# arkworks-rs/groth16

Hardware: AMD Instinct MI355X
Metric: R1CS constraints/sec (create_proof, BLS12-381) (higher is better)
Workload: dtype u32-limb Montgomery integers (Fr 255-bit, Fq 381-bit); 1 GPU; SYN(k=22) synthetic R1CS, 4194302 constraints, FFT domain 2^22, bls12_381, full create_proof (7 NTTs + 4 G1 MSMs + 1 G2 MSM), valid proving key generated on the GPU from seeded toxic waste; curve=bls12_381, log2_domain=22, constraints=4194302, key=valid, witness=resident in HBM at entry (--full: value_incl_h2d holds the PCIe-inclusive rates), parallelism=single-gpu

## Files before the change

groth16_amd/csrc/fp30.hpp:

```cpp
#pragma once
#include "field.hpp"
#include "fips_asm_gen.hpp"

#if defined(__HIP_DEVICE_COMPILE__) && !defined(G16_NO_FIPS_ASM)
#define G16_ASM_PRODUCTS 1
#endif

namespace g16 {

template <class P>
struct Fp30 {
    typedef P Params_t;
    static constexpr int NL = P::NL30;
    static constexpr int NW = P::N;
    static constexpr uint32_t MASK = (1u << 30) - 1u;
    uint32_t l[NL];

    G16_HD static Fp30 zero() {
        Fp30 r;
        G16_UNROLL for (int i = 0; i < NL; ++i) r.l[i] = 0;
        return r;
    }
    G16_HD static Fp30 one() {
        Fp30 r;
// ... 351 lines not shown
        }
        Fp30 r;
        const bool lt = br < 0;
        G16_UNROLL for (int i = 0; i < NL; ++i) r.l[i] = lt ? l[i] : d.l[i];
        return r;
    }
    G16_HD Fp30 weak_reduce32() const { return cond_sub<16>().template cond_sub<8>().template cond_sub<4>().template cond_sub<2>(); }
    G16_HD bool raw_zero() const {
        uint32_t a = 0;
        G16_UNROLL for (int i = 0; i < NL; ++i) a |= l[i];
        return a == 0;
    }
    typedef Fp30 Raw;
    static constexpr int KM = 2, K2M = 4, KX = 8, KY = 4;
#ifndef G16_ACC_MIN_WAVES
#define G16_ACC_MIN_WAVES 2
#endif
    static constexpr int ACC_MIN_WAVES = G16_ACC_MIN_WAVES;
    static constexpr bool ACC_PREFETCH = true;
    static constexpr int LANES_PER_TASK = 1;
    template <class A>
    G16_HD static bool load_point(const A* bases, int64_t idx, Fp30& px, Fp30& py) {
        const A p = bases[idx];
        if (p.is_identity()) return false;
        px = from_packed(p.x);
        py = from_packed(p.y);
        return true;
    }
    template <class A>
    G16_HD static bool load_point_py(const A* bases, int64_t idx, Fp30& px, PackedC& yw) {
        const A p = bases[idx];
        if (p.is_identity()) return false;
        px = from_packed(p.x);
        yw = p.y;
        return true;
    }


    G16_HD Fp30 canonical_lt2p() const {
        Fp30 d;
        int32_t br = 0;
        G16_UNROLL for (int i = 0; i < NL; ++i) {
            const int32_t v = (int32_t)l[i] - (int32_t)P::p30(i) + br;
            if (i == NL - 1) { d.l[i] = (uint32_t)v; br = v >> 31; }
            else { d.l[i] = (uint32_t)v & MASK; br = v >> 30; }
        }
        Fp30 r;
        const bool lt = br < 0;
        G16_UNROLL for (int i = 0; i < NL; ++i) r.l[i] = lt ? l[i] : d.l[i];
        return r;
    }

    G16_HD Fp30 canonical_lt8p() const { return cond_sub<4>().template cond_sub<2>().canonical_lt2p(); }
    G16_HD Fp30 canonical_quick() const {
        constexpr uint32_t D = P::p30(NL - 1) + 1u;
        static_assert(D > (1u << 13), "the top limb of p carries at least 14 bits for every supported field");
        constexpr uint64_t MAGIC = ((uint64_t)1 << 40) / D;
        const uint32_t q = (uint32_t)(((uint64_t)l[NL - 1] * MAGIC) >> 40);
        Fp30 r;
        int64_t carry = 0;
        G16_UNROLL for (int i = 0; i < NL; ++i) {
            const int64_t t = (int64_t)l[i] - (int64_t)((uint64_t)q * P::p30(i)) + carry;
            r.l[i] = (i == NL - 1) ? (uint32_t)t : ((uint32_t)t & MASK);
            carry = t >> 30;
        }
        return r.canonical_lt8p();
    }
    G16_HD Fp30 neg_canonical() const {
        Fp30 d;
        int32_t br = 0;
        G16_UNROLL for (int i = 0; i < NL; ++i) {
            const int32_t v = (int32_t)P::p30(i) - (int32_t)l[i] + br;
            if (i == NL - 1) d.l[i] = (uint32_t)v;
            else { d.l[i] = (uint32_t)v & MASK; br = v >> 30; }
        }
        return d;
    }
    G16_HD bool same_limbs(const Fp30& o) const {
        uint32_t a = 0;
        G16_UNROLL for (int i = 0; i < NL; ++i) a |= l[i] ^ o.l[i];
        return a == 0;
    }
    static constexpr int PREFIX_LIMBS = NL;
    G16_HD void get_limbs(uint32_t* w) const { G16_UNROLL for (int i = 0; i < NL; ++i) w[i] = l[i]; }
    G16_HD static Fp30 from_limbs(const uint32_t* w) { Fp30 r; G16_UNROLL for (int i = 0; i < NL; ++i) r.l[i] = w[i]; return r; }
    G16_HD bool equals_canonical(const Fp30& o) const { return same_limbs(o); }
    template <class A>
    G16_HD static void store_point(A* dst, int64_t idx, const Fp30& x, const Fp30& y, bool identity) {
        A p;
        if (identity) { p = A::identity(); }
        else { x.pack(p.x.v); y.pack(p.y.v); }
        dst[idx] = p;
    }

    G16_HD Std to_packed() const {
        Std r;
        mul_impl(one()).canonical_lt2p().pack(r.v);
        return r;
    }
    G16_HD static Fp<P> std_to_r30(const Fp<P>& x) {
        Fp<P> c;
        G16_UNROLL for (int i = 0; i < P::N; ++i) c.v[i] = P::r30_plain(i);
        return x * c;
    }
    G16_HD Fp<P> to_std() const {
        Fp30 c;
// ... 548 lines not shown
```

groth16_amd/csrc/hosttest.hip:

```cpp
#include "internal.hpp"
#include "fp30.hpp"
#include "batch_affine.hpp"
#include "window_tables.hpp"
#include "fixed_base.hpp"
#include <cstdlib>
#include <vector>

using namespace g16;

namespace g16 {
template <class P>
struct Fp2e30 {
    typedef Fp30<P> B;
    typedef Fp2p30<P> PP;
    B c0, c1;
    static Fp2e30 one() { return {B::one(), B::zero()}; }
    Fp2e30 add(const Fp2e30& o) const { return {c0.add(o.c0), c1.add(o.c1)}; }
    Fp2e30 dbl() const { return {c0.dbl(), c1.dbl()}; }
    template <int K> Fp2e30 sub(const Fp2e30& o) const { return {c0.template sub<K>(o.c0), c1.template sub<K>(o.c1)}; }
    Fp2e30 mul(const Fp2e30& o) const { return {PP::pair_mul(false, c0, c1, o.c0, o.c1), PP::pair_mul(true, c1, c0, o.c1, o.c0)}; }
    Fp2e30 sqr() const { return {PP::pair_sqr(false, c0, c1), PP::pair_sqr(true, c1, c0)}; }
};
template <class P>
Fp2e30<P> batch_inverse(const Fp2e30<P>& a) { return {pair_inverse<P>(false, a.c0, a.c1), pair_inverse<P>(true, a.c1, a.c0)}; }
// ... 87 lines not shown
    }
    static Fq rand_fq(uint64_t& st) {
        Fq acc = Fq::zero();
        const Fq two64 = Fq::from_u64(1ULL << 32).sqr();
        for (int k = 0; k < 8; ++k) acc = acc * two64 + Fq::from_u64(sm_next(st));
        return acc;
    }
    typedef Fp30<typename Fq::Params> F30;
    static F30 to30(const Fq& x) { const Fq t = F30::std_to_r30(x); return F30::unpack(t.v); }
    static Fr rand_fr(uint64_t& st) {
        Fr acc = Fr::zero();
        const Fr two64 = Fr::from_u64(1ULL << 32).sqr();
        for (int k = 0; k < 8; ++k) acc = acc * two64 + Fr::from_u64(sm_next(st));
        return acc;
    }
    static int selftest_fr30(uint64_t seed, int iters) {
        typedef Fp30<typename Fr::Params> R30;
        uint64_t st = seed ^ 0xF7;
        {
            R30 pl, kp = R30::zero();
            for (int i = 0; i < R30::NL; ++i) pl.l[i] = Fr::Params::p30(i);
            R30 pm1 = pl;
            pm1.l[0] -= 1;
            R30 one_raw = R30::zero();
            one_raw.l[0] = 1;
            for (int k = 0; k <= 5000; ++k) {
                if (k % 7 == 0 || k < 40 || (k & (k - 1)) == 0 || ((k + 1) & k) == 0) {
                    if (!kp.canonical_quick().same_limbs(R30::zero())) return 520;
                    if (!kp.add(pm1).canonical_quick().same_limbs(pm1)) return 521;
                    if (!kp.add(one_raw).canonical_quick().same_limbs(one_raw)) return 522;
                }
                kp = kp.add(pl);
            }
        }
        for (int it = 0; it < iters; ++it) {
            Fr x = rand_fr(st), y = rand_fr(st), w = rand_fr(st);
            if (it == 0) { x = Fr::zero(); }
            if (it == 1) { x = Fr::zero() - Fr::one(); y = x; w = x; }
            const R30 a = R30::unpack(x.v), b = R30::unpack(y.v);
            const Fr wt = R30::std_to_r30(w);
            const R30 w30 = R30::unpack(wt.v);
            auto canon = [](const R30& v) { Fr o; v.mul_impl(R30::one()).canonical_lt2p().pack(o.v); return o; };
            auto quick = [](const R30& v) { Fr o; v.canonical_quick().pack(o.v); return o; };
            if (!(canon(a.mul_impl(w30)) == x * w)) return 501;
            if (!(quick(a.mul_impl(w30)) == x * w) || !(quick(a) == x) || !(quick(R30::zero()) == Fr::zero())) return 505;
            {
                R30 m = R30::unpack((Fr::zero() - Fr::one()).v);
                Fr want = Fr::zero() - Fr::one();
                for (int k = 0; k < 12; ++k) {
                    if (!(quick(m) == want) || !(quick(m.add(R30::unpack(Fr::one().v))) == want + Fr::one())) return 506;
                    m = m.dbl(); want = want + want;
                }
            }
            R30 u = a, v = b;
            Fr ru = x, rv = y;
            for (int k = 0; k < 11; ++k) {
                const R30 t = v.mul_impl(w30);
                const R30 nu = u.add(t), nv = u.template sub<2>(t);
                const Fr rt = rv * w;
                const Fr rnu = ru + rt, rnv = ru - rt;
                u = nu; v = nv; ru = rnu; rv = rnv;
            }
            if (!(canon(u) == ru) || !(canon(v) == rv)) return 502;
            if (!(quick(u) == ru) || !(quick(v) == rv)) return 507;
            u = a; v = b; ru = x; rv = y;
            R30 s2 = a, d2 = b;
            for (int k = 0; k < 11; ++k) {
                const R30 nu = u.add(v);
                const R30 nv = u.sub_pow2(v, k).mul_impl(w30);
                const Fr rnu = ru + rv, rnv = (ru - rv) * w;
                s2 = nu; d2 = nv;
                u = nu; v = nu.add(nv).sub_pow2(nv, k + 1 < 12 ? k + 1 : 11);
                ru = rnu; rv = rnu;
                if (!(canon(d2) == rnv)) return 503;
                if (!(quick(d2) == rnv) || !(quick(nu) == rnu) || !(quick(v) == rnu)) return 508;
            }
            if (!(canon(s2) == ru)) return 504;
        }
        return 0;
    }

    template <class X, class A>
    static int selftest_fixed_base(const A& gen, uint64_t seed, int first_code) {
        uint64_t st = seed ^ 0xFB;
        uint32_t k0[8];
        for (int i = 0; i < 8; ++i) k0[i] = (uint32_t)sm_next(st);
        k0[7] &= 0x0fffffffu;
        const X p = X::from_affine(gen).mul_bits(k0, 256);
        FixedBaseTable<X> tab;
        tab.build(p);
        for (int it = 0; it < 6; ++it) {
            uint32_t k[8];
            for (int i = 0; i < 8; ++i) k[i] = it == 0 ? 0u : it == 1 ? (i == 0 ? 1u : 0u) : it == 2 ? 0xffffffffu : (uint32_t)sm_next(st);
            if (it == 3) for (int i = 0; i < Fr::N; ++i) k[i] = Fr::Params::mod(i) - (i == 0 ? 1u : 0u);
            const auto want = p.mul_bits(k, 256).to_affine();
            if (!(tab.mul(k).to_affine() == want)) return first_code;
            if (!(mul_window4(p, k).to_affine() == want)) return first_code + 1;
        }
        return 0;
    }

    template <class R30>
    static int selftest_columns(uint64_t seed, int iters) {
        typedef unsigned __int128 U128;
        uint64_t st = seed ^ 0xC0;
        for (int it = 0; it < iters + 4; ++it) {
// ... 495 lines not shown
```

groth16_amd/csrc/internal.hpp:

```cpp
#pragma once
#include <hip/hip_runtime.h>
#include <atomic>
#include <cstdint>
#include <cstdio>
#include <cstring>
#include <string>
#include <vector>
#include "../../include/g16_mi355x.h"
#include "curve.hpp"

namespace g16 {

void set_last_error(const char* what, hipError_t e, const char* file, int line);

#define G16_HIP_TRY(expr)                                                     \
    do {                                                                      \
        hipError_t e__ = (expr);                                              \
        if (e__ != hipSuccess) {                                              \
            ::g16::set_last_error(#expr, e__, __FILE__, __LINE__);            \
            return e__ == hipErrorOutOfMemory ? G16_ERR_OOM : G16_ERR_HIP;    \
        }                                                                     \
    } while (0)

#define G16_TRY(expr)                  \
// ... 4 lines not shown

#define G16_LAUNCH_CHECK() G16_HIP_TRY(hipGetLastError())

struct PerDeviceOnce {
    std::atomic<bool> done[64] = {};
    std::atomic<bool>& flag() {
        int dev = 0;
        (void)hipGetDevice(&dev);
        return done[dev & 63];
    }
};

struct Arena {
    struct Chunk { char* p; size_t cap; size_t used; };
    std::vector<Chunk> chunks;
    size_t min_chunk = (size_t)256 << 20;
    void reset() { for (auto& c : chunks) c.used = 0; }
    int alloc(size_t bytes, void** out);
    template <class T> int alloc_n(size_t n, T** out) { return alloc(n * sizeof(T), (void**)out); }
    void release();
    size_t total() const { size_t t = 0; for (auto& c : chunks) t += c.cap; return t; }
};

struct EventTimer {
    hipEvent_t a = nullptr, b = nullptr;
    bool used = false;
    int start(hipStream_t s) {
        if (!a) { G16_HIP_TRY(hipEventCreate(&a)); G16_HIP_TRY(hipEventCreate(&b)); }
        used = true;
        G16_HIP_TRY(hipEventRecord(a, s));
        return G16_OK;
    }
    int stop(hipStream_t s) { G16_HIP_TRY(hipEventRecord(b, s)); return G16_OK; }
    double ms() {
        if (!used) return 0.0;
        float t = 0.f;
        if (hipEventElapsedTime(&t, a, b) != hipSuccess) return 0.0;
        return (double)t;
    }
    void destroy() { if (a) { (void)hipEventDestroy(a); (void)hipEventDestroy(b); a = b = nullptr; } }
};

template <class C>
struct Domain {
    typedef typename C::Fr Fr;
    int log_n = 0;
    size_t n = 0;
    Fr* tw_fwd = nullptr;
    Fr* tw_inv = nullptr;
    Fr* s1_br = nullptr;
    Fr* s2 = nullptr;
    Fr* g_pow = nullptr;
    Fr n_inv, zinv;
};
template <class C> int domain_create(int log_n, hipStream_t st, Domain<C>** out);
template <class C> void domain_destroy(Domain<C>* d);
template <class C> int domain_ensure_gpow(Domain<C>* d, hipStream_t st);

template <class C> int ntt_dif(const Domain<C>* d, typename C::Fr* data, bool inverse, hipStream_t st);
template <class C> int ntt_dif_quotient(const Domain<C>* d, typename C::Fr* a, const typename C::Fr* b, const typename C::Fr* c,
                                        const typename C::Fr& zinv, bool inverse, hipStream_t st);
template <class C> int ntt_dit(const Domain<C>* d, typename C::Fr* data, bool inverse, const typename C::Fr* prescale, hipStream_t st);
template <class C> int ntt_dif_dit(const Domain<C>* d, typename C::Fr* data, bool dif_inverse, const typename C::Fr* prescale, hipStream_t st);
template <class C> int ntt_dif_batch(const Domain<C>* d, typename C::Fr* const* data, int nbatch, bool inverse, hipStream_t st);
template <class C> int ntt_dit_batch(const Domain<C>* d, typename C::Fr* const* data, int nbatch, bool inverse, const typename C::Fr* prescale,
                                     hipStream_t st);
template <class C> int ntt_dif_dit_batch(const Domain<C>* d, typename C::Fr* const* data, int nbatch, bool dif_inverse,
                                         const typename C::Fr* prescale, hipStream_t st);
template <class C> int bitrev_scale(const Domain<C>* d, typename C::Fr* out, const typename C::Fr* in, const typename C::Fr* table,
                                    const typename C::Fr* cst, hipStream_t st);
template <class C> int scale_by_table(typename C::Fr* data, const typename C::Fr* table, size_t n, hipStream_t st);
template <class C> int gen_power_table(typename C::Fr* out, size_t n, const typename C::Fr& base, const typename C::Fr& scale, bool r30_form,
                                       hipStream_t st);

template <class C>
struct DeviceCircuit {
    typedef typename C::Fr Fr;
    uint64_t num_inputs = 0, num_constraints = 0, num_variables = 0;
    uint64_t* row_ptr[3] = {nullptr, nullptr, nullptr};
    uint32_t* col[3] = {nullptr, nullptr, nullptr};
    Fr* val[3] = {nullptr, nullptr, nullptr};
    uint64_t nnz[3] = {0, 0, 0};
    Domain<C>* dom = nullptr;
    static constexpr int Z_CHUNKS = 8;
    uint64_t need_col[Z_CHUNKS] = {};
};
struct ZUpload {
    const void* host = nullptr;
    hipStream_t copy_stream = nullptr;
    hipEvent_t landed[8] = {};
    int pieces = 0;
};
template <class C> int mark_unit_coefficients(DeviceCircuit<C>* ck, hipStream_t st);
template <class C> int witness_map_device(const DeviceCircuit<C>* ck, const typename C::Fr* d_z, typename C::Fr* d_h, Arena& arena,
                                          hipStream_t st, EventTimer* ntt_timers = nullptr, ZUpload* up = nullptr);

template <class C>
struct DistWm {
    typedef typename C::Fr Fr;
    int rank = 0, world = 1, log_world = 0;
    size_t M = 0, blk = 0;
    Domain<C>* dom_m = nullptr;
    Fr* tw1 = nullptr;
    Fr* sc_mid = nullptr;
    Fr* tw2 = nullptr;
    Fr* sc_out = nullptr;
    Fr wn_fwd[8], wn_inv[8];
    Fr zinv;
};
template <class C> int dwm_create(const DeviceCircuit<C>* ck, int rank, int world, hipStream_t st, DistWm<C>** out);
template <class C> void dwm_destroy(DistWm<C>* d);
template <class C> int dwm_stage(const DeviceCircuit<C>* ck, const DistWm<C>* dw, int stage, const typename C::Fr* d_z,
                                 typename C::Fr* const work[3], typename C::Fr* const recv[3], typename C::Fr* h_local, hipStream_t st);

struct MsmPlan {
    int c = 0;
    int W = 0;
    int groups = 0;
    bool merged = false;
    uint32_t B = 0;
    uint32_t Lmax = 0;
    int affine_levels = 0;
    uint32_t chunk = 0;
// ... 75 lines not shown
```

groth16_amd/csrc/ntt.hip:

```cpp
#include "internal.hpp"
#include "fp30.hpp"

namespace g16 {

#ifndef G16_NTT_TILE_LOG
#define G16_NTT_TILE_LOG 10
#endif
static constexpr int NTT_TILE_LOG = G16_NTT_TILE_LOG;
static constexpr int NTT_TILE = 1 << NTT_TILE_LOG;
#ifdef G16_NTT_THREADS
static constexpr int NTT_THREADS = G16_NTT_THREADS;
#else
static constexpr int NTT_THREADS = NTT_TILE_LOG >= 12 ? 512 : 256;
#endif
#ifndef G16_NTT_MAX_R
#define G16_NTT_MAX_R 2
#endif
static constexpr int NTT_MAX_R = G16_NTT_MAX_R;
#ifndef G16_NTT_MIN_WAVES
#define G16_NTT_MIN_WAVES 4
#endif
static constexpr int NTT_MAX_STRIDED = NTT_TILE_LOG >= 12 ? 10 : 8;
static constexpr int NTT_ROW = NTT_TILE + NTT_TILE / 32;

// ... 85 lines not shown
        G16_UNROLL for (int j = 0; j < NE; ++j) {
            const uint32_t c = lds_col(ebase | ((uint32_t)j << p0));
            G16_UNROLL for (int l = 0; l < NL; ++l) lds[l * NTT_ROW + c] = x[j].l[l];
        }
    }
}

template <class P>
struct NttBatch { Fp<P>* p[3]; };
template <class P>
struct NttQuot { const Fp<P>* b; const Fp<P>* c; Fp<P> zinv; };

template <class P, bool DIT>
__global__ __launch_bounds__(NTT_THREADS, G16_NTT_MIN_WAVES) void ntt30_pass_kernel(NttBatch<P> batch, const Tw<P>* __restrict__ tw,
                                                                 const Fp<P>* __restrict__ prescale, int log_n, int s_lo, int s_hi,
                                                                 int T, NttQuot<P> quot) {
    typedef Fp30<P> F;
    constexpr int NL = F::NL;
    extern __shared__ __attribute__((aligned(16))) unsigned char smem[];
    uint32_t* lds = reinterpret_cast<uint32_t*>(smem);
    Fp<P>* __restrict__ data = batch.p[blockIdx.y];
    const int K = s_hi - s_lo;
    const int TT = (s_lo == 0) ? 0 : T;
    const uint32_t E = 1u << (K + TT);
    const uint64_t blk = blockIdx.x;
    uint64_t base;
    if (s_lo == 0) {
        base = blk << K;
    } else {
        const int mid_bits = s_lo - T;
        const uint64_t lowpart = blk & ((1ull << mid_bits) - 1);
        const uint64_t hipart = blk >> mid_bits;
        base = (lowpart << T) | (hipart << s_hi);
    }
    auto gidx = [&](uint32_t e) -> uint64_t {
        if (s_lo == 0) return base + e;
        const uint32_t low = e & ((1u << T) - 1), mid = e >> T;
        return base + low + ((uint64_t)mid << s_lo);
    };
    auto lds_load = [&](uint32_t e) -> F {
        F x;
        const uint32_t c = lds_col(e);
        G16_UNROLL for (int l = 0; l < NL; ++l) x.l[l] = lds[l * NTT_ROW + c];
        return x;
    };
    auto lds_store = [&](uint32_t e, const F& x) {
        const uint32_t c = lds_col(e);
        G16_UNROLL for (int l = 0; l < NL; ++l) lds[l * NTT_ROW + c] = x.l[l];
    };
    for (uint32_t e = threadIdx.x; e < E; e += NTT_THREADS) {
        const uint64_t g = gidx(e);
        F x;
        if (quot.b) {
            const Fp<P> t = (data[g] * quot.b[g] - quot.c[g]) * quot.zinv;
            x = F::unpack(t.v);
        } else {
            x = F::unpack(data[g].v);
        }
        if (prescale) x = x.mul_impl(F::unpack(prescale[g].v));
        lds_store(e, x);
    }
    __syncthreads();
    int done = 0;
    while (done < K) {
        const int R = (K - done) >= NTT_MAX_R ? NTT_MAX_R : (K - done);
        const int q0 = DIT ? done : (K - done - R);
        if (R == 3) ntt30_round<P, DIT, 3>(lds, tw, log_n, s_lo, q0, TT, E, done, gidx, true);
        else if (R == 2) ntt30_round<P, DIT, 2>(lds, tw, log_n, s_lo, q0, TT, E, done, gidx, true);
        else ntt30_round<P, DIT, 1>(lds, tw, log_n, s_lo, q0, TT, E, done, gidx, true);
        __syncthreads();
        done += R;
    }
    for (uint32_t e = threadIdx.x; e < E; e += NTT_THREADS) {
        const F x = lds_load(e).canonical_quick();
        Fp<P> o;
        x.pack(o.v);
        data[gidx(e)] = o;
    }
}

template <class P>
__global__ __launch_bounds__(NTT_THREADS, G16_NTT_MIN_WAVES) void ntt30_dif_dit_kernel(NttBatch<P> batch, const Tw<P>* __restrict__ tw_dif,
                                                                    const Tw<P>* __restrict__ tw_dit, const Fp<P>* __restrict__ prescale,
                                                                    int log_n, int K) {
    typedef Fp30<P> F;
    constexpr int NL = F::NL;
    extern __shared__ __attribute__((aligned(16))) unsigned char smem[];
    uint32_t* lds = reinterpret_cast<uint32_t*>(smem);
    Fp<P>* __restrict__ data = batch.p[blockIdx.y];
    const uint32_t E = 1u << K;
    const uint64_t base = (uint64_t)blockIdx.x << K;
    auto gidx = [&](uint32_t e) -> uint64_t { return base + e; };
    for (uint32_t e = threadIdx.x; e < E; e += NTT_THREADS) {
        const F x = F::unpack(data[base + e].v);
        const uint32_t c = lds_col(e);
        G16_UNROLL for (int l = 0; l < NL; ++l) lds[l * NTT_ROW + c] = x.l[l];
    }
    __syncthreads();
    for (int done = 0; done < K;) {
        const int R = (K - done) >= NTT_MAX_R ? NTT_MAX_R : (K - done);
        const int q0 = K - done - R;
        if (R == 3) ntt30_round<P, false, 3>(lds, tw_dif, log_n, 0, q0, 0, E, done, gidx, true);
        else if (R == 2) ntt30_round<P, false, 2>(lds, tw_dif, log_n, 0, q0, 0, E, done, gidx, true);
        else ntt30_round<P, false, 1>(lds, tw_dif, log_n, 0, q0, 0, E, done, gidx, true);
        __syncthreads();
        done += R;
    }
    if (prescale) {
        for (uint32_t e = threadIdx.x; e < E; e += NTT_THREADS) {
            const uint32_t c = lds_col(e);
            F x;
            G16_UNROLL for (int l = 0; l < NL; ++l) x.l[l] = lds[l * NTT_ROW + c];
            x = x.mul_impl(F::unpack(prescale[base + e].v));
            G16_UNROLL for (int l = 0; l < NL; ++l) lds[l * NTT_ROW + c] = x.l[l];
        }
        __syncthreads();
    }
    for (int done = 0; done < K;) {
        const int R = (K - done) >= NTT_MAX_R ? NTT_MAX_R : (K - done);
        const bool unit0 = prescale != nullptr;
        if (R == 3) ntt30_round<P, true, 3>(lds, tw_dit, log_n, 0, done, 0, E, done, gidx, unit0);
        else if (R == 2) ntt30_round<P, true, 2>(lds, tw_dit, log_n, 0, done, 0, E, done, gidx, unit0);
        else ntt30_round<P, true, 1>(lds, tw_dit, log_n, 0, done, 0, E, done, gidx, unit0);
        __syncthreads();
        done += R;
    }
    for (uint32_t e = threadIdx.x; e < E; e += NTT_THREADS) {
        const uint32_t c = lds_col(e);
        F x;
        G16_UNROLL for (int l = 0; l < NL; ++l) x.l[l] = lds[l * NTT_ROW + c];
        Fp<P> o;
        x.canonical_quick().pack(o.v);
        data[base + e] = o;
    }
}

template <class P>
__global__ void bitrev_scale_kernel(Fp<P>* __restrict__ out, const Fp<P>* __restrict__ in, const Fp<P>* __restrict__ table, Fp<P> cst,
                                    int has_cst, int log_n) {
    typedef Fp30<P> F;
    size_t k = (size_t)blockIdx.x * blockDim.x + threadIdx.x;
    if (k >= ((size_t)1 << log_n)) return;
    Fp<P> o = in[bitrev32((uint32_t)k, log_n)];
    if (table || has_cst) {
        F x = F::unpack(o.v);
        if (table) x = x.mul_impl(F::unpack(table[k].v));
        if (has_cst) x = x.mul_impl(F::unpack(cst.v));
        x.canonical_lt2p().pack(o.v);
    }
    out[k] = o;
}

template <class P>
__global__ void scale_table_kernel(Fp<P>* __restrict__ data, const Fp<P>* __restrict__ table, size_t n) {
    typedef Fp30<P> F;
    size_t k = (size_t)blockIdx.x * blockDim.x + threadIdx.x;
    if (k >= n) return;
    Fp<P> o;
    F::unpack(data[k].v).mul_impl(F::unpack(table[k].v)).canonical_lt2p().pack(o.v);
    data[k] = o;
}

struct PassPlan { int s_lo, s_hi, T; };

static std::vector<PassPlan> plan_passes(int log_n) {
    std::vector<PassPlan> p;
    if (log_n <= NTT_TILE_LOG) {
        p.push_back({0, log_n, 0});
        return p;
    }
    p.push_back({0, NTT_TILE_LOG, 0});
    int rest = log_n - NTT_TILE_LOG;
    const int npass = (rest + NTT_MAX_STRIDED - 1) / NTT_MAX_STRIDED;
    int s = NTT_TILE_LOG;
    for (int i = 0; i < npass; ++i) {
        const int left = npass - i;
        const int k = (rest + left - 1) / left;
        p.push_back({s, s + k, NTT_TILE_LOG - k});
        s += k;
        rest -= k;
    }
    return p;
}

template <class P, bool DIT>
static int launch_pass(const NttBatch<P>& batch, int nbatch, const Tw<P>* tw, const Fp<P>* prescale, int log_n, const PassPlan& pp, hipStream_t st,
                       const NttQuot<P>* quot = nullptr) {
    const int K = pp.s_hi - pp.s_lo;
    const int TT = pp.s_lo == 0 ? 0 : pp.T;
    const size_t E = (size_t)1 << (K + TT);
    const size_t blocks = ((size_t)1 << log_n) / E;
    const size_t lds_bytes = (size_t)Fp30<P>::NL * NTT_ROW * sizeof(uint32_t);
    static PerDeviceOnce attr_once;
    std::atomic<bool>& attr_set = attr_once.flag();
    if (!attr_set) {
        G16_HIP_TRY(hipFuncSetAttribute(reinterpret_cast<const void*>(&ntt30_pass_kernel<P, DIT>),
                                        hipFuncAttributeMaxDynamicSharedMemorySize, (int)lds_bytes));
        attr_set = true;
    }
    NttQuot<P> q;
    if (quot) q = *quot;
    else { q.b = nullptr; q.c = nullptr; q.zinv = Fp<P>::zero(); }
// ... 11 lines not shown
}

template <class C>
int ntt_dif_batch(const Domain<C>* d, typename C::Fr* const* data, int nbatch, bool inverse, hipStream_t st) {
    typedef typename C::Fr::Params P;
    if (nbatch < 1 || nbatch > 3) return G16_ERR_INTERNAL;
    if (d->log_n == 0) return G16_OK;
    auto passes = plan_passes(d->log_n);
    const Tw<P>* tw = reinterpret_cast<const Tw<P>*>(inverse ? d->tw_inv : d->tw_fwd);
    const NttBatch<P> b = make_batch<C>(data, nbatch);
    for (size_t i = passes.size(); i-- > 0;) G16_TRY((launch_pass<P, false>(b, nbatch, tw, nullptr, d->log_n, passes[i], st)));
    return G16_OK;
}
template <class C>
int ntt_dif(const Domain<C>* d, typename C::Fr* data, bool inverse, hipStream_t st) { return ntt_dif_batch<C>(d, &data, 1, inverse, st); }

template <class C>
int ntt_dif_quotient(const Domain<C>* d, typename C::Fr* a, const typename C::Fr* b, const typename C::Fr* c, const typename C::Fr& zinv,
                     bool inverse, hipStream_t st) {
    typedef typename C::Fr::Params P;
    auto passes = plan_passes(d->log_n);
    const Tw<P>* tw = reinterpret_cast<const Tw<P>*>(inverse ? d->tw_inv : d->tw_fwd);
    typename C::Fr* data[1] = {a};
    const NttBatch<P> batch = make_batch<C>(data, 1);
    NttQuot<P> q;
    q.b = b; q.c = c; q.zinv = zinv;
    if (d->log_n == 0) return G16_ERR_INTERNAL;
    for (size_t i = passes.size(); i-- > 0;)
        G16_TRY((launch_pass<P, false>(batch, 1, tw, nullptr, d->log_n, passes[i], st, i + 1 == passes.size() ? &q : nullptr)));
    return G16_OK;
}

template <class C>
int ntt_dit_batch(const Domain<C>* d, typename C::Fr* const* data, int nbatch, bool inverse, const typename C::Fr* prescale, hipStream_t st) {
    typedef typename C::Fr::Params P;
    if (nbatch < 1 || nbatch > 3) return G16_ERR_INTERNAL;
    if (d->log_n == 0) {
        if (prescale) for (int i = 0; i < nbatch; ++i) G16_TRY((scale_by_table<C>(data[i], prescale, 1, st)));
        return G16_OK;
    }
    auto passes = plan_passes(d->log_n);
    const Tw<P>* tw = reinterpret_cast<const Tw<P>*>(inverse ? d->tw_inv : d->tw_fwd);
    const NttBatch<P> b = make_batch<C>(data, nbatch);
    for (size_t i = 0; i < passes.size(); ++i)
        G16_TRY((launch_pass<P, true>(b, nbatch, tw, i == 0 ? prescale : nullptr, d->log_n, passes[i], st)));
    return G16_OK;
}
template <class C>
int ntt_dit(const Domain<C>* d, typename C::Fr* data, bool inverse, const typename C::Fr* prescale, hipStream_t st) {
    return ntt_dit_batch<C>(d, &data, 1, inverse, prescale, st);
}

template <class C>
int ntt_dif_dit_batch(const Domain<C>* d, typename C::Fr* const* data, int nbatch, bool dif_inverse, const typename C::Fr* prescale, hipStream_t st) {
    typedef typename C::Fr::Params P;
    if (nbatch < 1 || nbatch > 3) return G16_ERR_INTERNAL;
    if (d->log_n == 0) {
        if (prescale) for (int i = 0; i < nbatch; ++i) G16_TRY((scale_by_table<C>(data[i], prescale, 1, st)));
        return G16_OK;
    }
    auto passes = plan_passes(d->log_n);
    const Tw<P>* tw1 = reinterpret_cast<const Tw<P>*>(dif_inverse ? d->tw_inv : d->tw_fwd);
    const Tw<P>* tw2 = reinterpret_cast<const Tw<P>*>(dif_inverse ? d->tw_fwd : d->tw_inv);
    const NttBatch<P> b = make_batch<C>(data, nbatch);
    for (size_t i = passes.size(); i-- > 1;) G16_TRY((launch_pass<P, false>(b, nbatch, tw1, nullptr, d->log_n, passes[i], st)));
    {
        const int K = passes[0].s_hi;
        const size_t blocks = ((size_t)1 << d->log_n) >> K;
        const size_t lds_bytes = (size_t)Fp30<P>::NL * NTT_ROW * sizeof(uint32_t);
        static PerDeviceOnce attr_once;
        std::atomic<bool>& attr_set = attr_once.flag();
        if (!attr_set) {
            G16_HIP_TRY(hipFuncSetAttribute(reinterpret_cast<const void*>(&ntt30_dif_dit_kernel<P>), hipFuncAttributeMaxDynamicSharedMemorySize,
                                            (int)lds_bytes));
            attr_set = true;
        }
        hipLaunchKernelGGL((ntt30_dif_dit_kernel<P>), dim3((unsigned)blocks, (unsigned)nbatch), dim3(NTT_THREADS), lds_bytes, st, b, tw1, tw2, prescale,
                           d->log_n, K);
        G16_LAUNCH_CHECK();
    }
    for (size_t i = 1; i < passes.size(); ++i) G16_TRY((launch_pass<P, true>(b, nbatch, tw2, nullptr, d->log_n, passes[i], st)));
    return G16_OK;
}
template <class C>
int ntt_dif_dit(const Domain<C>* d, typename C::Fr* data, bool dif_inverse, const typename C::Fr* prescale, hipStream_t st) {
    return ntt_dif_dit_batch<C>(d, &data, 1, dif_inverse, prescale, st);
}

template <class C>
int bitrev_scale(const Domain<C>* d, typename C::Fr* out, const typename C::Fr* in, const typename C::Fr* table,
                 const typename C::Fr* cst, hipStream_t st) {
    typedef typename C::Fr Fr;
    const size_t n = d->n;
    Fr c = cst ? *cst : Fr::zero();
    hipLaunchKernelGGL((bitrev_scale_kernel<typename Fr::Params>), dim3((unsigned)((n + 255) / 256)), dim3(256), 0, st, out, in, table, c,
                       cst ? 1 : 0, d->log_n);
    G16_LAUNCH_CHECK();
    return G16_OK;
}

template <class C>
int scale_by_table(typename C::Fr* data, const typename C::Fr* table, size_t n, hipStream_t st) {
    typedef typename C::Fr Fr;
    hipLaunchKernelGGL((scale_table_kernel<typename Fr::Params>), dim3((unsigned)((n + 255) / 256)), dim3(256), 0, st, data, table, n);
    G16_LAUNCH_CHECK();
    return G16_OK;
}

template <class Fr>
static int gen_powers30(Fr* out, size_t n, const Fr& base, const Fr& scale, int rev_bits, hipStream_t st, int layered_log = 0) {
    if (n == 0) return G16_OK;
    PowTable<Fr> tab;
    Fr p = base;
    for (int j = 0; j < 32; ++j) { tab.p[j] = p; p = p.sqr(); }
    const Fr scale30 = Fp30<typename Fr::Params>::std_to_r30(scale);
    hipLaunchKernelGGL((gen_powers_kernel<Fr>), dim3((unsigned)((n + 255) / 256)), dim3(256), 0, st, out, n, tab, scale30, rev_bits, layered_log);
    G16_LAUNCH_CHECK();
    return G16_OK;
}

template <class C>
int gen_power_table(typename C::Fr* out, size_t n, const typename C::Fr& base, const typename C::Fr& scale, bool r30_form, hipStream_t st) {
    typedef typename C::Fr Fr;
    if (r30_form) return gen_powers30<Fr>(out, n, base, scale, 0, st);
    if (n == 0) return G16_OK;
    PowTable<Fr> tab;
    Fr p = base;
    for (int j = 0; j < 32; ++j) { tab.p[j] = p; p = p.sqr(); }
    hipLaunchKernelGGL((gen_powers_kernel<Fr>), dim3((unsigned)((n + 255) / 256)), dim3(256), 0, st, out, n, tab, scale, 0, 0);
    G16_LAUNCH_CHECK();
    return G16_OK;
}

template <class C>
int domain_create(int log_n, hipStream_t st, Domain<C>** out) {
    typedef typename C::Fr Fr;
    if (log_n > C::TWO_ADICITY || log_n > 31) return G16_ERR_DEGREE_TOO_LARGE;
    Domain<C>* d = new Domain<C>();
    d->log_n = log_n;
    d->n = (size_t)1 << log_n;
    const size_t n = d->n;
    Fr omega = C::two_adic_root();
    for (int i = log_n; i < C::TWO_ADICITY; ++i) omega = omega.sqr();
    Fr omega_inv = omega.inverse();
    const Fr n_inv = Fr::from_u64((uint64_t)n).inverse();
    d->n_inv = Fp30<typename Fr::Params>::std_to_r30(n_inv);
    const Fr g = C::fr_generator(), g_inv = C::fr_generator_inv();
    d->zinv = (g.pow_u64((uint64_t)n) - Fr::one()).inverse();
    int rc = G16_OK;
    const size_t ntw = n > 1 ? n - 1 : 1;
    typedef Tw<typename Fr::Params> TwE;
    Fr* tw_tmp = nullptr;
    auto fail = [&](int code) {
        (void)hipStreamSynchronize(st);
        (void)hipFree(tw_tmp);
        domain_destroy<C>(d);
        return code;
    };
    if (hipMalloc((void**)&d->tw_fwd, ntw * sizeof(TwE)) != hipSuccess) return fail(G16_ERR_OOM);
    if (hipMalloc((void**)&d->tw_inv, ntw * sizeof(TwE)) != hipSuccess) return fail(G16_ERR_OOM);
    if (hipMalloc((void**)&tw_tmp, ntw * sizeof(Fr)) != hipSuccess) return fail(G16_ERR_OOM);
    if (hipMalloc((void**)&d->s1_br, n * sizeof(Fr)) != hipSuccess) return fail(G16_ERR_OOM);
    if (hipMalloc((void**)&d->s2, n * sizeof(Fr)) != hipSuccess) return fail(G16_ERR_OOM);
    for (int dir = 0; dir < 2; ++dir) {
        if ((rc = gen_powers30<Fr>(tw_tmp, ntw, dir ? omega_inv : omega, Fr::one(), 0, st, log_n)) != G16_OK) return fail(rc);
        hipLaunchKernelGGL((tw_convert_kernel<typename Fr::Params>), dim3((unsigned)((ntw + 255) / 256)), dim3(256), 0, st, tw_tmp,
                           reinterpret_cast<TwE*>(dir ? d->tw_inv : d->tw_fwd), ntw);
        if (hipGetLastError() != hipSuccess) return fail(G16_ERR_HIP);
    }
    if ((rc = gen_powers30<Fr>(d->s1_br, n, g, n_inv, log_n, st)) != G16_OK) return fail(rc);
    if ((rc = gen_powers30<Fr>(d->s2, n, g_inv, n_inv, 0, st)) != G16_OK) return fail(rc);
    if (hipStreamSynchronize(st) != hipSuccess) return fail(G16_ERR_HIP);
    (void)hipFree(tw_tmp);
    *out = d;
    return G16_OK;
}

template <class C>
int domain_ensure_gpow(Domain<C>* d, hipStream_t st) {
    typedef typename C::Fr Fr;
    if (d->g_pow) return G16_OK;
    G16_HIP_TRY(hipMalloc((void**)&d->g_pow, d->n * sizeof(Fr)));
    return gen_powers30<Fr>(d->g_pow, d->n, C::fr_generator(), Fr::one(), 0, st);
}

template <class C>
void domain_destroy(Domain<C>* d) {
    if (!d) return;
    (void)hipFree(d->tw_fwd); (void)hipFree(d->tw_inv); (void)hipFree(d->s1_br); (void)hipFree(d->s2); (void)hipFree(d->g_pow);
    delete d;
}

#define G16_INSTANTIATE_NTT(C)                                                                                     \
    template int domain_create<C>(int, hipStream_t, Domain<C>**);                                                  \
    template void domain_destroy<C>(Domain<C>*);                                                                   \
    template int domain_ensure_gpow<C>(Domain<C>*, hipStream_t);                                                   \
    template int ntt_dif<C>(const Domain<C>*, typename C::Fr*, bool, hipStream_t);                                 \
    template int ntt_dif_quotient<C>(const Domain<C>*, typename C::Fr*, const typename C::Fr*, const typename C::Fr*, const typename C::Fr&, bool, hipStream_t); \
    template int ntt_dit<C>(const Domain<C>*, typename C::Fr*, bool, const typename C::Fr*, hipStream_t);          \
    template int ntt_dif_dit<C>(const Domain<C>*, typename C::Fr*, bool, const typename C::Fr*, hipStream_t);      \
    template int ntt_dif_batch<C>(const Domain<C>*, typename C::Fr* const*, int, bool, hipStream_t);              \
    template int ntt_dit_batch<C>(const Domain<C>*, typename C::Fr* const*, int, bool, const typename C::Fr*, hipStream_t);   \
    template int ntt_dif_dit_batch<C>(const Domain<C>*, typename C::Fr* const*, int, bool, const typename C::Fr*, hipStream_t); \
    template int bitrev_scale<C>(const Domain<C>*, typename C::Fr*, const typename C::Fr*, const typename C::Fr*,  \
                                 const typename C::Fr*, hipStream_t);                                              \
    template int scale_by_table<C>(typename C::Fr*, const typename C::Fr*, size_t, hipStream_t);                   \
    template int gen_power_table<C>(typename C::Fr*, size_t, const typename C::Fr&, const typename C::Fr&, bool, hipStream_t);

G16_INSTANTIATE_NTT(Bls12_381)
G16_INSTANTIATE_NTT(Bn254)

}
```

groth16_amd/csrc/witness_map.hip:

```cpp
#include "internal.hpp"
#include <algorithm>
#include <new>

namespace g16 {

template <class Fr>
struct SpmvArgs {
    const uint64_t* row_ptr[3];
    const uint32_t* col[3];
    const Fr* val[3];
    Fr* out[3];
};

template <class Fr>
__global__ void spmv3_kernel(SpmvArgs<Fr> args, const Fr* __restrict__ z, uint64_t num_inputs, uint64_t nc, uint64_t row0, uint64_t stride,
                             uint64_t rows, int out_rev_bits, uint64_t out0) {
    const int m = blockIdx.y;
    const uint64_t li = (uint64_t)blockIdx.x * blockDim.x + threadIdx.x;
    if (li >= rows) return;
    const uint64_t row = row0 + stride * li;
    Fr acc = Fr::zero();
    if (row < nc) {
        const uint64_t b = args.row_ptr[m][row], e = args.row_ptr[m][row + 1];
        const Fr one = Fr::one();
// ... 23 lines not shown
template <class C>
int witness_map_device(const DeviceCircuit<C>* ck, const typename C::Fr* d_z, typename C::Fr* d_h, Arena& arena, hipStream_t st,
                       EventTimer* ntt_timers, ZUpload* up) {
    typedef typename C::Fr Fr;
    const Domain<C>* dom = ck->dom;
    const size_t n = dom->n;
    Fr *a = nullptr, *b = nullptr, *c = nullptr;
    G16_TRY(arena.alloc_n(n, &a));
    G16_TRY(arena.alloc_n(n, &b));
    G16_TRY(arena.alloc_n(n, &c));
    SpmvArgs<Fr> args;
    Fr* outs[3] = {a, b, c};
    for (int m = 0; m < 3; ++m) {
        args.row_ptr[m] = ck->row_ptr[m];
        args.col[m] = ck->col[m];
        args.val[m] = ck->val[m];
        args.out[m] = outs[m];
    }
    if (!up) {
        hipLaunchKernelGGL((spmv3_kernel<Fr>), dim3((unsigned)((n + 255) / 256), 3), dim3(256), 0, st, args, d_z, ck->num_inputs,
                           ck->num_constraints, (uint64_t)0, (uint64_t)1, (uint64_t)n, 0, (uint64_t)0);
        G16_LAUNCH_CHECK();
    } else {
        constexpr int ZC = DeviceCircuit<C>::Z_CHUNKS;
        const uint64_t nz = ck->num_variables;
        const int pieces = (int)std::min<uint64_t>(4, std::max<uint64_t>(1, nz >> 16));
        up->pieces = pieces;
        const uint64_t per = (nz + pieces - 1) / pieces;
        for (int k = 0; k < pieces; ++k) {
            const uint64_t lo = per * k, hi = std::min(nz, per * (k + 1));
            if (hi > lo)
                G16_HIP_TRY(hipMemcpyAsync(const_cast<Fr*>(d_z) + lo, static_cast<const Fr*>(up->host) + lo, (hi - lo) * sizeof(Fr),
                                           hipMemcpyHostToDevice, up->copy_stream));
            G16_HIP_TRY(hipEventRecord(up->landed[k], up->copy_stream));
        }
        int next_block = 0;
        for (int k = 0; k < pieces; ++k) {
            const uint64_t hi = std::min(nz, per * (k + 1));
            int last_block = next_block;
            while (last_block < ZC && (k == pieces - 1 || ck->need_col[last_block] < hi)) ++last_block;
            if (last_block > next_block) {
                const uint64_t r_lo = n * (uint64_t)next_block / ZC, r_hi = n * (uint64_t)last_block / ZC;
                G16_HIP_TRY(hipStreamWaitEvent(st, up->landed[k], 0));
                if (r_hi > r_lo) {
                    hipLaunchKernelGGL((spmv3_kernel<Fr>), dim3((unsigned)((r_hi - r_lo + 255) / 256), 3), dim3(256), 0, st, args, d_z, ck->num_inputs,
                                       ck->num_constraints, r_lo, (uint64_t)1, r_hi - r_lo, 0, r_lo);
                    G16_LAUNCH_CHECK();
                }
                next_block = last_block;
            }
        }
    }
    if (ntt_timers) G16_TRY(ntt_timers[0].start(st));
    G16_TRY((ntt_dif_dit_batch<C>(dom, outs, 3, true, dom->s1_br, st)));
    if (ntt_timers) G16_TRY(ntt_timers[0].stop(st));
    if (ntt_timers) G16_TRY(ntt_timers[1].start(st));
    if (dom->log_n == 0) {
        hipLaunchKernelGGL((quotient_kernel<Fr>), dim3((unsigned)((n + 255) / 256)), dim3(256), 0, st, a, b, c, dom->zinv, n);
        G16_LAUNCH_CHECK();
    } else {
        G16_TRY((ntt_dif_quotient<C>(dom, a, b, c, dom->zinv, true, st)));
    }
    G16_TRY((bitrev_scale<C>(dom, d_h, a, dom->s2, nullptr, st)));
    if (ntt_timers) G16_TRY(ntt_timers[1].stop(st));
    return G16_OK;
}

template <class Fr>
struct SmallRoots { Fr w[8]; };

template <class Fr, int LOGN>
__device__ __forceinline__ void dft_small(Fr* v, const SmallRoots<Fr>& roots) {
    constexpr int N = 1 << LOGN;
    G16_UNROLL for (int s = LOGN - 1; s >= 0; --s) {
        const int half = 1 << s;
        G16_UNROLL for (int i = 0; i < N; ++i) {
            if (i & half) continue;
            const int k = (i & (half - 1)) << (LOGN - 1 - s);
            const Fr u = v[i], t = v[i + half];
            v[i] = u + t;
            v[i + half] = k ? (u - t) * roots.w[k] : (u - t);
        }
    }
    G16_UNROLL for (int i = 0; i < N; ++i) {
        int j = 0;
        G16_UNROLL for (int b = 0; b < LOGN; ++b) j |= ((i >> b) & 1) << (LOGN - 1 - b);
        if (j > i) { const Fr t = v[i]; v[i] = v[j]; v[j] = t; }
    }
}

template <class Fr, int LOGN, bool TWO>
__global__ __launch_bounds__(128) void dwm_column_kernel(const Fr* __restrict__ in0, const Fr* __restrict__ in1, const Fr* __restrict__ in2, Fr* __restrict__ out0,
                                  Fr* __restrict__ out1, Fr* __restrict__ out2, size_t blk, SmallRoots<Fr> roots_a, const Fr* __restrict__ sc_a,
                                  SmallRoots<Fr> roots_b, const Fr* __restrict__ sc_b) {
    constexpr int N = 1 << LOGN;
    const size_t j = (size_t)blockIdx.x * blockDim.x + threadIdx.x;
    if (j >= blk) return;
    const Fr* in = blockIdx.y == 0 ? in0 : blockIdx.y == 1 ? in1 : in2;
    Fr* out = blockIdx.y == 0 ? out0 : blockIdx.y == 1 ? out1 : out2;
    Fr v[N];
    G16_UNROLL for (int i = 0; i < N; ++i) v[i] = in[(size_t)i * blk + j];
    dft_small<Fr, LOGN>(v, roots_a);
    G16_UNROLL for (int i = 0; i < N; ++i) v[i] = v[i] * sc_a[(size_t)i * blk + j];
    if (TWO) {
        dft_small<Fr, LOGN>(v, roots_b);
        G16_UNROLL for (int i = 0; i < N; ++i) v[i] = v[i] * sc_b[(size_t)i * blk + j];
    }
    G16_UNROLL for (int i = 0; i < N; ++i) out[(size_t)i * blk + j] = v[i];
}

template <class C>
void dwm_destroy(DistWm<C>* d) {
    if (!d) return;
    (void)hipFree(d->tw1); (void)hipFree(d->sc_mid); (void)hipFree(d->tw2); (void)hipFree(d->sc_out);
    domain_destroy<C>(d->dom_m);
    delete d;
// ... 139 lines not shown
```

Before: 67.42 million constraints/s.

## Skip coset round-trip of C polynomial by subtracting it in the final scaling

Uses linearity of the inverse NTT: C is only inverse-transformed (DIF step), while its coset forward DIT passes are skipped. The quotient then computes A*B*zinv alone, and the final bitrev-scale kernel subtracts C scaled by zinv/n at the end. This removes one full forward NTT over 2^22 elements and the later inverse work attributed to C, at the cost of an extra read and multiply in the bitrev kernel. Correctness relies on the coset scaling tables lining up algebraically.

After: 67.43 million constraints/s (median of 2 runs). No clear change (+0.0%).

```diff
diff --git a/groth16_amd/csrc/fp30.hpp b/groth16_amd/csrc/fp30.hpp
--- a/groth16_amd/csrc/fp30.hpp
+++ b/groth16_amd/csrc/fp30.hpp
@@ -427,6 +427,9 @@
     }
 
     G16_HD Fp30 canonical_lt8p() const { return cond_sub<4>().template cond_sub<2>().canonical_lt2p(); }
+    G16_HD static Fp30 mul_sub_canonical(const Fp30& a, const Fp30& t, const Fp30& b, const Fp30& c) {
+        return a.mul_impl(t).template sub<2>(b.mul_impl(c)).canonical_lt8p();
+    }
     G16_HD Fp30 canonical_quick() const {
         constexpr uint32_t D = P::p30(NL - 1) + 1u;
         static_assert(D > (1u << 13), "the top limb of p carries at least 14 bits for every supported field");
diff --git a/groth16_amd/csrc/hosttest.hip b/groth16_amd/csrc/hosttest.hip
--- a/groth16_amd/csrc/hosttest.hip
+++ b/groth16_amd/csrc/hosttest.hip
@@ -163,6 +163,28 @@
                     m = m.dbl(); want = want + want;
                 }
             }
+            {
+                auto unperm = [](const R30& xa, const R30& ta, const R30& ya, const R30& ca) {
+                    Fr o;
+                    R30::mul_sub_canonical(xa, ta, ya, ca).pack(o.v);
+                    return o;
+                };
+                const Fr cc = rand_fr(st), m1 = Fr::zero() - Fr::one();
+                const Fr cct = R30::std_to_r30(cc), m1t = R30::std_to_r30(m1);
+                const R30 c30 = R30::unpack(cct.v), pm = R30::unpack(m1.v), pmt = R30::unpack(m1t.v), z30 = R30::zero();
+                if (!(unperm(a, w30, b, c30) == x * w - y * cc)) return 509;
+                if (!(unperm(pm, pmt, pm, pmt) == Fr::zero())) return 510;
+                if (!(unperm(z30, pmt, pm, pmt) == Fr::zero() - Fr::one())) return 511;
+                if (!(unperm(pm, pmt, z30, pmt) == Fr::one())) return 512;
+                if (!(unperm(pm, pmt, pm, R30::unpack(R30::std_to_r30(Fr::one()).v)) == Fr::one() + Fr::one())) return 513;
+                if (!(unperm(a, w30, a, w30) == Fr::zero())) return 514;
+                R30 top;
+                for (int i = 0; i < R30::NL; ++i) top.l[i] = Fr::Params::p30(i);
+                top.l[0] -= 1;
+                const Fr sq = quick(top.mul_impl(top));
+                if (!(unperm(top, top, top, top) == Fr::zero())) return 515;
+                if (!(unperm(top, top, z30, top) == sq) || !(unperm(z30, top, top, top) == Fr::zero() - sq)) return 516;
+            }
             R30 u = a, v = b;
             Fr ru = x, rv = y;
             for (int k = 0; k < 11; ++k) {
diff --git a/groth16_amd/csrc/internal.hpp b/groth16_amd/csrc/internal.hpp
--- a/groth16_amd/csrc/internal.hpp
+++ b/groth16_amd/csrc/internal.hpp
@@ -80,6 +80,7 @@
     Fr* s2 = nullptr;
     Fr* g_pow = nullptr;
     Fr n_inv, zinv;
+    Fr zinv_n_inv;
 };
 template <class C> int domain_create(int log_n, hipStream_t st, Domain<C>** out);
 template <class C> void domain_destroy(Domain<C>* d);
@@ -94,9 +95,11 @@
 template <class C> int ntt_dit_batch(const Domain<C>* d, typename C::Fr* const* data, int nbatch, bool inverse, const typename C::Fr* prescale,
                                      hipStream_t st);
 template <class C> int ntt_dif_dit_batch(const Domain<C>* d, typename C::Fr* const* data, int nbatch, bool dif_inverse,
-                                         const typename C::Fr* prescale, hipStream_t st);
+                                         const typename C::Fr* prescale, int dif_only, hipStream_t st);
 template <class C> int bitrev_scale(const Domain<C>* d, typename C::Fr* out, const typename C::Fr* in, const typename C::Fr* table,
                                     const typename C::Fr* cst, hipStream_t st);
+template <class C> int bitrev_scale_sub(const Domain<C>* d, typename C::Fr* out, const typename C::Fr* in, const typename C::Fr* table,
+                                        const typename C::Fr* sub, const typename C::Fr& cst2, hipStream_t st);
 template <class C> int scale_by_table(typename C::Fr* data, const typename C::Fr* table, size_t n, hipStream_t st);
 template <class C> int gen_power_table(typename C::Fr* out, size_t n, const typename C::Fr& base, const typename C::Fr& scale, bool r30_form,
                                        hipStream_t st);
diff --git a/groth16_amd/csrc/ntt.hip b/groth16_amd/csrc/ntt.hip
--- a/groth16_amd/csrc/ntt.hip
+++ b/groth16_amd/csrc/ntt.hip
@@ -161,7 +161,8 @@
         const uint64_t g = gidx(e);
         F x;
         if (quot.b) {
-            const Fp<P> t = (data[g] * quot.b[g] - quot.c[g]) * quot.zinv;
+            const Fp<P> ab = data[g] * quot.b[g];
+            const Fp<P> t = (quot.c ? ab - quot.c[g] : ab) * quot.zinv;
             x = F::unpack(t.v);
         } else {
             x = F::unpack(data[g].v);
@@ -191,7 +192,7 @@
 template <class P>
 __global__ __launch_bounds__(NTT_THREADS, G16_NTT_MIN_WAVES) void ntt30_dif_dit_kernel(NttBatch<P> batch, const Tw<P>* __restrict__ tw_dif,
                                                                     const Tw<P>* __restrict__ tw_dit, const Fp<P>* __restrict__ prescale,
-                                                                    int log_n, int K) {
+                                                                    int log_n, int K, int full_chains) {
     typedef Fp30<P> F;
     constexpr int NL = F::NL;
     extern __shared__ __attribute__((aligned(16))) unsigned char smem[];
@@ -215,24 +216,26 @@
         __syncthreads();
         done += R;
     }
-    if (prescale) {
-        for (uint32_t e = threadIdx.x; e < E; e += NTT_THREADS) {
-            const uint32_t c = lds_col(e);
-            F x;
-            G16_UNROLL for (int l = 0; l < NL; ++l) x.l[l] = lds[l * NTT_ROW + c];
-            x = x.mul_impl(F::unpack(prescale[base + e].v));
-            G16_UNROLL for (int l = 0; l < NL; ++l) lds[l * NTT_ROW + c] = x.l[l];
-        }
-        __syncthreads();
-    }
-    for (int done = 0; done < K;) {
-        const int R = (K - done) >= NTT_MAX_R ? NTT_MAX_R : (K - done);
-        const bool unit0 = prescale != nullptr;
-        if (R == 3) ntt30_round<P, true, 3>(lds, tw_dit, log_n, 0, done, 0, E, done, gidx, unit0);
-        else if (R == 2) ntt30_round<P, true, 2>(lds, tw_dit, log_n, 0, done, 0, E, done, gidx, unit0);
-        else ntt30_round<P, true, 1>(lds, tw_dit, log_n, 0, done, 0, E, done, gidx, unit0);
-        __syncthreads();
-        done += R;
+    if ((int)blockIdx.y < full_chains) {
+        if (prescale) {
+            for (uint32_t e = threadIdx.x; e < E; e += NTT_THREADS) {
+                const uint32_t c = lds_col(e);
+                F x;
+                G16_UNROLL for (int l = 0; l < NL; ++l) x.l[l] = lds[l * NTT_ROW + c];
+                x = x.mul_impl(F::unpack(prescale[base + e].v));
+                G16_UNROLL for (int l = 0; l < NL; ++l) lds[l * NTT_ROW + c] = x.l[l];
+            }
+            __syncthreads();
+        }
+        for (int done = 0; done < K;) {
+            const int R = (K - done) >= NTT_MAX_R ? NTT_MAX_R : (K - done);
+            const bool unit0 = prescale != nullptr;
+            if (R == 3) ntt30_round<P, true, 3>(lds, tw_dit, log_n, 0, done, 0, E, done, gidx, unit0);
+            else if (R == 2) ntt30_round<P, true, 2>(lds, tw_dit, log_n, 0, done, 0, E, done, gidx, unit0);
+            else ntt30_round<P, true, 1>(lds, tw_dit, log_n, 0, done, 0, E, done, gidx, unit0);
+            __syncthreads();
+            done += R;
+        }
     }
     for (uint32_t e = threadIdx.x; e < E; e += NTT_THREADS) {
         const uint32_t c = lds_col(e);
@@ -257,6 +260,18 @@
         if (has_cst) x = x.mul_impl(F::unpack(cst.v));
         x.canonical_lt2p().pack(o.v);
     }
+    out[k] = o;
+}
+
+template <class P>
+__global__ void bitrev_scale_sub_kernel(Fp<P>* __restrict__ out, const Fp<P>* __restrict__ in, const Fp<P>* __restrict__ table,
+                                        const Fp<P>* __restrict__ sub, Fp<P> cst2, int log_n) {
+    typedef Fp30<P> F;
+    size_t k = (size_t)blockIdx.x * blockDim.x + threadIdx.x;
+    if (k >= ((size_t)1 << log_n)) return;
+    const uint32_t r = bitrev32((uint32_t)k, log_n);
+    Fp<P> o;
+    F::mul_sub_canonical(F::unpack(in[r].v), F::unpack(table[k].v), F::unpack(sub[r].v), F::unpack(cst2.v)).pack(o.v);
     out[k] = o;
 }
 
@@ -374,11 +389,13 @@
 }
 
 template <class C>
-int ntt_dif_dit_batch(const Domain<C>* d, typename C::Fr* const* data, int nbatch, bool dif_inverse, const typename C::Fr* prescale, hipStream_t st) {
+int ntt_dif_dit_batch(const Domain<C>* d, typename C::Fr* const* data, int nbatch, bool dif_inverse, const typename C::Fr* prescale, int dif_only,
+                      hipStream_t st) {
     typedef typename C::Fr::Params P;
-    if (nbatch < 1 || nbatch > 3) return G16_ERR_INTERNAL;
+    if (nbatch < 1 || nbatch > 3 || dif_only < 0 || dif_only > nbatch) return G16_ERR_INTERNAL;
+    const int nfull = nbatch - dif_only;
     if (d->log_n == 0) {
-        if (prescale) for (int i = 0; i < nbatch; ++i) G16_TRY((scale_by_table<C>(data[i], prescale, 1, st)));
+        if (prescale) for (int i = 0; i < nfull; ++i) G16_TRY((scale_by_table<C>(data[i], prescale, 1, st)));
         return G16_OK;
     }
     auto passes = plan_passes(d->log_n);
@@ -398,15 +415,16 @@
             attr_set = true;
         }
         hipLaunchKernelGGL((ntt30_dif_dit_kernel<P>), dim3((unsigned)blocks, (unsigned)nbatch), dim3(NTT_THREADS), lds_bytes, st, b, tw1, tw2, prescale,
-                           d->log_n, K);
+                           d->log_n, K, nfull);
         G16_LAUNCH_CHECK();
     }
-    for (size_t i = 1; i < passes.size(); ++i) G16_TRY((launch_pass<P, true>(b, nbatch, tw2, nullptr, d->log_n, passes[i], st)));
+    if (nfull > 0)
+        for (size_t i = 1; i < passes.size(); ++i) G16_TRY((launch_pass<P, true>(b, nfull, tw2, nullptr, d->log_n, passes[i], st)));
     return G16_OK;
 }
 template <class C>
 int ntt_dif_dit(const Domain<C>* d, typename C::Fr* data, bool dif_inverse, const typename C::Fr* prescale, hipStream_t st) {
-    return ntt_dif_dit_batch<C>(d, &data, 1, dif_inverse, prescale, st);
+    return ntt_dif_dit_batch<C>(d, &data, 1, dif_inverse, prescale, 0, st);
 }
 
 template <class C>
@@ -417,6 +435,17 @@
     Fr c = cst ? *cst : Fr::zero();
     hipLaunchKernelGGL((bitrev_scale_kernel<typename Fr::Params>), dim3((unsigned)((n + 255) / 256)), dim3(256), 0, st, out, in, table, c,
                        cst ? 1 : 0, d->log_n);
+    G16_LAUNCH_CHECK();
+    return G16_OK;
+}
+
+template <class C>
+int bitrev_scale_sub(const Domain<C>* d, typename C::Fr* out, const typename C::Fr* in, const typename C::Fr* table,
+                     const typename C::Fr* sub, const typename C::Fr& cst2, hipStream_t st) {
+    typedef typename C::Fr Fr;
+    const size_t n = d->n;
+    hipLaunchKernelGGL((bitrev_scale_sub_kernel<typename Fr::Params>), dim3((unsigned)((n + 255) / 256)), dim3(256), 0, st, out, in, table, sub,
+                       cst2, d->log_n);
     G16_LAUNCH_CHECK();
     return G16_OK;
 }
@@ -469,6 +498,7 @@
     d->n_inv = Fp30<typename Fr::Params>::std_to_r30(n_inv);
     const Fr g = C::fr_generator(), g_inv = C::fr_generator_inv();
     d->zinv = (g.pow_u64((uint64_t)n) - Fr::one()).inverse();
+    d->zinv_n_inv = Fp30<typename Fr::Params>::std_to_r30(d->zinv * n_inv);
     int rc = G16_OK;
     const size_t ntw = n > 1 ? n - 1 : 1;
     typedef Tw<typename Fr::Params> TwE;
@@ -523,7 +553,9 @@
     template int ntt_dif_dit<C>(const Domain<C>*, typename C::Fr*, bool, const typename C::Fr*, hipStream_t);      \
     template int ntt_dif_batch<C>(const Domain<C>*, typename C::Fr* const*, int, bool, hipStream_t);              \
     template int ntt_dit_batch<C>(const Domain<C>*, typename C::Fr* const*, int, bool, const typename C::Fr*, hipStream_t);   \
-    template int ntt_dif_dit_batch<C>(const Domain<C>*, typename C::Fr* const*, int, bool, const typename C::Fr*, hipStream_t); \
+    template int ntt_dif_dit_batch<C>(const Domain<C>*, typename C::Fr* const*, int, bool, const typename C::Fr*, int, hipStream_t); \
+    template int bitrev_scale_sub<C>(const Domain<C>*, typename C::Fr*, const typename C::Fr*, const typename C::Fr*,  \
+                                     const typename C::Fr*, const typename C::Fr&, hipStream_t);                   \
     template int bitrev_scale<C>(const Domain<C>*, typename C::Fr*, const typename C::Fr*, const typename C::Fr*,  \
                                  const typename C::Fr*, hipStream_t);                                              \
     template int scale_by_table<C>(typename C::Fr*, const typename C::Fr*, size_t, hipStream_t);                   \
diff --git a/groth16_amd/csrc/witness_map.hip b/groth16_amd/csrc/witness_map.hip
--- a/groth16_amd/csrc/witness_map.hip
+++ b/groth16_amd/csrc/witness_map.hip
@@ -99,16 +99,17 @@
         }
     }
     if (ntt_timers) G16_TRY(ntt_timers[0].start(st));
-    G16_TRY((ntt_dif_dit_batch<C>(dom, outs, 3, true, dom->s1_br, st)));
+    G16_TRY((ntt_dif_dit_batch<C>(dom, outs, 3, true, dom->s1_br, 1, st)));
     if (ntt_timers) G16_TRY(ntt_timers[0].stop(st));
     if (ntt_timers) G16_TRY(ntt_timers[1].start(st));
     if (dom->log_n == 0) {
         hipLaunchKernelGGL((quotient_kernel<Fr>), dim3((unsigned)((n + 255) / 256)), dim3(256), 0, st, a, b, c, dom->zinv, n);
         G16_LAUNCH_CHECK();
+        G16_TRY((bitrev_scale<C>(dom, d_h, a, dom->s2, nullptr, st)));
     } else {
-        G16_TRY((ntt_dif_quotient<C>(dom, a, b, c, dom->zinv, true, st)));
-    }
-    G16_TRY((bitrev_scale<C>(dom, d_h, a, dom->s2, nullptr, st)));
+        G16_TRY((ntt_dif_quotient<C>(dom, a, b, nullptr, dom->zinv, true, st)));
+        G16_TRY((bitrev_scale_sub<C>(dom, d_h, a, dom->s2, c, dom->zinv_n_inv, st)));
+    }
     if (ntt_timers) G16_TRY(ntt_timers[1].stop(st));
     return G16_OK;
 }
```
